# hpcaitech/Open-Sora

Hardware: NVIDIA H100
Metric: denoise-steps/sec STDiT3-XL/2 64x32x32 bf16 (higher is better)
Workload: dtype bf16

## Files before the change

### open-sora_b200/csrc/gemm_sm90.cu

```cuda
#include <stdlib.h>

#include <type_traits>

#include "common.cuh"
#include "tiles.cuh"
#include "wgmma.cuh"

namespace osb {

constexpr int kBlockM = 128;
constexpr int kBlockK = 64;
constexpr int kNumThreads = 384;
constexpr int kStageBudget = 200 * 1024;
constexpr int kSmemLimit = 227 * 1024;

enum { kPlain = 0, kConv = 1, kHeadTiles = 2, kLora = 3, kText = 4, kFp8 = 5, kFp8Blk = 6 };

struct Fp8BlockParams {
  int64_t a_ld, a_kstride;
  uint8_t* d8;
  float* d_scale;
  int64_t ldd8, ld_dscale;
};

// ... 31 lines not shown
  int32_t kw_n, kh_n;
  int32_t cin_chunks;
};

__host__ __device__ constexpr bool staged_epilogue(int mode) { return mode == kPlain || mode == kConv || mode == kLora || mode == kFp8 || mode == kFp8Blk; }

template <int BLOCK_N, bool kStaged = false>
struct GemmCfg {
  static constexpr int A_BYTES = kBlockM * kBlockK * 2;
  static constexpr int B_BYTES = BLOCK_N * kBlockK * 2;
  static constexpr int STAGE_BYTES = A_BYTES + B_BYTES;
  static constexpr int EPI_BYTES = kStaged ? kBlockM * BLOCK_N * 2 : 0;
  static constexpr int RING_BUDGET = kStaged ? kSmemLimit - 1024 - 256 - EPI_BYTES : kStageBudget;
  static constexpr int STAGES_RAW = RING_BUDGET / STAGE_BYTES;
  static constexpr int STAGES = STAGES_RAW > 6 ? 6 : STAGES_RAW;
  static constexpr int NUM_BARS = 2 * STAGES + (kStaged ? 1 : 0);
  static constexpr int SMEM_BYTES = STAGES * STAGE_BYTES + EPI_BYTES + 1024 + 8 * NUM_BARS;
  static_assert(STAGES >= 2, "pipeline needs at least two stages");
  static_assert(SMEM_BYTES <= kSmemLimit, "shared memory");
  static_assert(B_BYTES % 1024 == 0, "W tile must keep 1024-byte swizzle-atom alignment");
  static_assert(BLOCK_N % 16 == 0 && BLOCK_N <= 256, "wgmma N");
  static_assert(!kStaged || BLOCK_N % 64 == 0, "the staged epilogue moves 64-column boxes");
};

template <int BLOCK_N, int kMode>
__global__ void __launch_bounds__(kNumThreads, 1)
gemm_bf16_kernel(const __grid_constant__ CUtensorMap tmap_a, const __grid_constant__ CUtensorMap tmap_w,
                 const GemmEpilogueParams p, const ConvGeom cg, const HeadTileParams ht,
                 const __grid_constant__ CUtensorMap tmap_u, const __grid_constant__ CUtensorMap tmap_lb,
                 const int32_t lora_k_blocks,
                 const float* a_scale, const float* w_scale,
                 const Fp8BlockParams fb,
                 const __grid_constant__ CUtensorMap tmap_r,
                 const __grid_constant__ CUtensorMap tmap_d) {
  constexpr bool kStaged = staged_epilogue(kMode);
  using Cfg = GemmCfg<BLOCK_N, kStaged>;
  constexpr int kStages = Cfg::STAGES;
  constexpr int kBK = (kMode == kFp8 || kMode == kFp8Blk) ? 2 * kBlockK : kBlockK;
  constexpr uint32_t kEpiBoxBytes = kBlockM * 128;

  extern __shared__ uint8_t smem_raw[];
  const uint32_t smem_base = (smem_u32(smem_raw) + 1023u) & ~1023u;
  const uint32_t epi_base = smem_base + kStages * Cfg::STAGE_BYTES;
  const uint32_t bar_base = epi_base + Cfg::EPI_BYTES;
  auto full_bar = [&](int s) { return bar_base + 8u * s; };
  auto empty_bar = [&](int s) { return bar_base + 8u * (kStages + s); };
  const uint32_t res_bar = bar_base + 8u * (2 * kStages);
  auto smem_a = [&](int s) { return smem_base + s * Cfg::STAGE_BYTES; };
  auto smem_b = [&](int s) { return smem_base + s * Cfg::STAGE_BYTES + Cfg::A_BYTES; };

  const int wg = threadIdx.x >> 7;
  const int tid_wg = threadIdx.x & 127;
  const int64_t num_n_blocks = (p.N + BLOCK_N - 1) / BLOCK_N;
  const int64_t m_blk = blockIdx.x / num_n_blocks, n_blk = blockIdx.x % num_n_blocks;
  const int64_t num_k_blocks = (p.K + kBK - 1) / kBK;
  const int64_t total_k_blocks = kMode == kLora ? num_k_blocks + lora_k_blocks : num_k_blocks;
  int n_i = 0, t0 = 0, h0 = 0, w0 = 0;
  if constexpr (kMode == kConv) {
    const int tw = (int)(m_blk % cg.tiles_w);
    const int th = (int)((m_blk / cg.tiles_w) % cg.tiles_h);
    const int tt = (int)((m_blk / ((int64_t)cg.tiles_w * cg.tiles_h)) % cg.tiles_t);
    n_i = (int)(m_blk / ((int64_t)cg.tiles_w * cg.tiles_h * cg.tiles_t));
    w0 = tw << cg.wt_log2;
    h0 = th << cg.ht_log2;
    t0 = tt * (128 >> (cg.wt_log2 + cg.ht_log2));
  }

  if (threadIdx.x == 0) {
    tma_prefetch_desc(&tmap_a);
    tma_prefetch_desc(&tmap_w);
    if constexpr (kMode == kLora) {
      tma_prefetch_desc(&tmap_u);
      tma_prefetch_desc(&tmap_lb);
    }
    if constexpr (kStaged) {
      if (p.R != nullptr) tma_prefetch_desc(&tmap_r);
      tma_prefetch_desc(&tmap_d);
      mbar_init(res_bar, 1);
    }
    for (int s = 0; s < kStages; ++s) {
      mbar_init(full_bar(s), 1);
      mbar_init(empty_bar(s), 2);
    }
    fence_barrier_init();
  }
  __syncthreads();
  pdl_wait();

  if (wg == 0) {
    if (tid_wg == 0) {
      const int32_t a_row = (int32_t)(m_blk * kBlockM);
      const int32_t w_row = (int32_t)(n_blk * BLOCK_N);
      if constexpr (kStaged) {
        if (p.R != nullptr) {
          const int live = (int)min((int64_t)(BLOCK_N / 64), (p.N - w_row + 63) / 64);
          mbar_expect_tx(res_bar, (uint32_t)live * kEpiBoxBytes);
          for (int c = 0; c < live; ++c) {
            if constexpr (kMode == kConv)
              tma_load_5d(&tmap_r, res_bar, epi_base + c * kEpiBoxBytes, w_row + 64 * c, w0, h0, t0, n_i);
            else
              tma_load_2d(&tmap_r, res_bar, epi_base + c * kEpiBoxBytes, w_row + 64 * c, a_row);
          }
        }
      }
      int stage = 0;
      uint32_t phase = 0;
      for (int64_t kb = 0; kb < num_k_blocks; ++kb) {
        mbar_wait_notrace(empty_bar(stage), phase ^ 1);
        const int32_t k0 = (int32_t)(kb * kBK);
        mbar_expect_tx(full_bar(stage), Cfg::STAGE_BYTES);
        if constexpr (kMode == kConv) {
          const int tap = (int)(kb / cg.cin_chunks);
          const int32_t ac = (int32_t)(kb - (int64_t)tap * cg.cin_chunks) * kBlockK;
          const int32_t aw = w0 * cg.sw + tap % cg.kw_n;
          const int32_t ah = h0 * cg.sh + (tap / cg.kw_n) % cg.kh_n;
          const int32_t at = t0 * cg.st + tap / (cg.kw_n * cg.kh_n);
          tma_load_5d(&tmap_a, full_bar(stage), smem_a(stage), ac, aw, ah, at, n_i);
        } else {
          tma_load_2d(&tmap_a, full_bar(stage), smem_a(stage), k0, a_row);
        }
        tma_load_2d(&tmap_w, full_bar(stage), smem_b(stage), k0, w_row);
        if (++stage == kStages) { stage = 0; phase ^= 1; }
      }
      if constexpr (kMode == kLora) {
        for (int32_t lk = 0; lk < lora_k_blocks; ++lk) {
          mbar_wait_notrace(empty_bar(stage), phase ^ 1);
          mbar_expect_tx(full_bar(stage), Cfg::STAGE_BYTES);
          tma_load_2d(&tmap_u, full_bar(stage), smem_a(stage), lk * kBlockK, a_row);
          tma_load_2d(&tmap_lb, full_bar(stage), smem_b(stage), lk * kBlockK, w_row);
          if (++stage == kStages) { stage = 0; phase ^= 1; }
        }
      }
      pdl_launch_dependents();
    }
    return;
  }

  const int cw = wg - 1;
  float acc[BLOCK_N / 2];
#pragma unroll
  for (int i = 0; i < BLOCK_N / 2; ++i) acc[i] = 0.f;
  if constexpr (kMode == kFp8 || kMode == kFp8Blk) {
    float part[BLOCK_N / 2];
#pragma unroll
    for (int i = 0; i < BLOCK_N / 2; ++i) part[i] = 0.f;
    const float* sa_row0 = a_scale;
    const float* sa_row1 = a_scale;
    if constexpr (kMode == kFp8Blk) {
      const int64_t r0 = m_blk * kBlockM + cw * 64 + (tid_wg >> 5) * 16 + ((tid_wg & 31) >> 2);
      sa_row0 = a_scale + min(r0, p.M - 1) * fb.a_ld;
      sa_row1 = a_scale + min(r0 + 8, p.M - 1) * fb.a_ld;
    }
    int stage = 0;
    uint32_t phase = 0;
    for (int64_t kb = 0; kb < total_k_blocks; ++kb) {
      float s0 = 1.f, s1 = 1.f;
      if constexpr (kMode == kFp8Blk) {
        s0 = __ldg(sa_row0 + kb * fb.a_kstride);
        s1 = __ldg(sa_row1 + kb * fb.a_kstride);
      }
      mbar_wait_notrace(full_bar(stage), phase);
      const uint64_t da = make_sw128_kmajor_desc(smem_a(stage) + (uint32_t)(cw * 64 * 128));
      const uint64_t db = make_sw128_kmajor_desc(smem_b(stage));
      wgmma_fence_regs(part);
      wgmma_fence();
#pragma unroll
      for (int k = 0; k < 4; ++k)
        WgmmaFp8<BLOCK_N>::mma(part, da + (uint64_t)(2 * k), db + (uint64_t)(2 * k), k > 0 ? 1u : 0u);
      wgmma_commit();
      wgmma_wait<0>();
      wgmma_fence_regs(part);
      if (tid_wg == 0) mbar_arrive(empty_bar(stage));
      if constexpr (kMode == kFp8Blk) {
#pragma unroll
        for (int j = 0; j < BLOCK_N / 8; ++j) {
          acc[4 * j] = fmaf(part[4 * j], s0, acc[4 * j]);
          acc[4 * j + 1] = fmaf(part[4 * j + 1], s0, acc[4 * j + 1]);
          acc[4 * j + 2] = fmaf(part[4 * j + 2], s1, acc[4 * j + 2]);
          acc[4 * j + 3] = fmaf(part[4 * j + 3], s1, acc[4 * j + 3]);
        }
      } else {
#pragma unroll
        for (int i = 0; i < BLOCK_N / 2; ++i) acc[i] += part[i];
      }
      if (++stage == kStages) { stage = 0; phase ^= 1; }
    }
  } else {
    int stage = 0, prev = 0;
    uint32_t phase = 0;
    for (int64_t kb = 0; kb < total_k_blocks; ++kb) {
      mbar_wait_notrace(full_bar(stage), phase);
      const uint64_t da = make_sw128_kmajor_desc(smem_a(stage) + (uint32_t)(cw * 64 * 128));
      const uint64_t db = make_sw128_kmajor_desc(smem_b(stage));
      wgmma_fence_regs(acc);
      wgmma_fence();
#pragma unroll
      for (int k = 0; k < kBlockK / 16; ++k)
        Wgmma<BLOCK_N>::mma(acc, da + (uint64_t)(2 * k), db + (uint64_t)(2 * k), (kb > 0 || k > 0) ? 1u : 0u);
      wgmma_commit();
      wgmma_wait<1>();
      wgmma_fence_regs(acc);
      if (kb > 0 && tid_wg == 0) mbar_arrive(empty_bar(prev));
      prev = stage;
      if (++stage == kStages) { stage = 0; phase ^= 1; }
    }
    wgmma_wait<0>();
    wgmma_fence_regs(acc);
  }

  const int warp_in = tid_wg >> 5, lane = tid_wg & 31;
  const int r_frag = cw * 64 + warp_in * 16 + (lane >> 2);
  const int c_frag = 2 * (lane & 3);

  if constexpr (kMode == kLora) {
    if (w_scale != nullptr) {
#pragma unroll
      for (int j = 0; j < BLOCK_N / 8; ++j) {
        const int64_t n = min(n_blk * BLOCK_N + 8 * j + c_frag, p.N - 2);
        const float2 cs = __ldg(reinterpret_cast<const float2*>(w_scale + n));
        acc[4 * j] *= cs.x;
        acc[4 * j + 1] *= cs.y;
        acc[4 * j + 2] *= cs.x;
        acc[4 * j + 3] *= cs.y;
      }
    }
  }

  if constexpr (kMode == kFp8Blk && BLOCK_N == 128) {
    if (p.epilogue == OSB_EPI_BIAS_GELU_TANH_FP8) {
      const int64_t n0 = n_blk * BLOCK_N + c_frag;
#pragma unroll
      for (int h = 0; h < 2; ++h) {
        const int64_t row = m_blk * kBlockM + r_frag + 8 * h;
        float amax = 0.f;
#pragma unroll
        for (int j = 0; j < BLOCK_N / 8; ++j) {
          const int64_t n = n0 + 8 * j;
          const float2 sw = __ldg(reinterpret_cast<const float2*>(w_scale + n));
          float v0 = acc[4 * j + 2 * h] * sw.x, v1 = acc[4 * j + 2 * h + 1] * sw.y;
          if (p.bias) {
            const float2 b = unpack_bf16x2(__ldg(reinterpret_cast<const uint32_t*>(p.bias + n)));
            v0 += b.x;
            v1 += b.y;
          }
          v0 = gelu_tanh(v0);
          v1 = gelu_tanh(v1);
          acc[4 * j + 2 * h] = v0;
          acc[4 * j + 2 * h + 1] = v1;
          amax = fmaxf(amax, fmaxf(fabsf(v0), fabsf(v1)));
        }
        amax = fmaxf(amax, __shfl_xor_sync(0xffffffffu, amax, 1));
        amax = fmaxf(amax, __shfl_xor_sync(0xffffffffu, amax, 2));
        const float s = amax > 0.f ? amax / 448.0f : 1.0f;
        if (row < p.M) {
          uint8_t* drow = fb.d8 + row * fb.ldd8;
#pragma unroll
          for (int j = 0; j < BLOCK_N / 8; ++j)
            *reinterpret_cast<uint16_t*>(drow + n0 + 8 * j) =
                (uint16_t)e4m3x2(acc[4 * j + 2 * h] / s, acc[4 * j + 2 * h + 1] / s);
          if (c_frag == 0) fb.d_scale[row * fb.ld_dscale + n_blk] = s;
        }
      }
      return;
    }
  }

  if constexpr (kMode == kHeadTiles) {
    constexpr int D = BLOCK_N / 2;
    using HT = HeadTileCfg<D>;
    constexpr int JH = D / 8;
    const int C = ht.heads * D;
    const uint32_t chunk_bytes = (uint32_t)ht.map.TR * 128u;
#pragma unroll
    for (int h = 0; h < 2; ++h) {
      const int64_t row = m_blk * kBlockM + r_frag + 8 * h;
      const bool row_ok = row < p.M;
      uint32_t pos = 0, tile_i = 0, seq;
      int r = 0;
      if (row_ok) {
        const uint32_t row32 = (uint32_t)row;
        if (ht.map.mode == 0) {
          seq = row32 / (uint32_t)ht.map.L;
          pos = row32 - seq * (uint32_t)ht.map.L;
        } else {
          const uint32_t ts = (uint32_t)ht.map.T * (uint32_t)ht.map.S;
          const uint32_t b = row32 / ts;
          const uint32_t rem = row32 - b * ts;
          pos = rem / (uint32_t)ht.map.S;
          seq = b * (uint32_t)ht.map.S + (rem - pos * (uint32_t)ht.map.S);
        }
        if (ht.map.G > 1) {
          tile_i = seq / (uint32_t)ht.map.G;
          r = (int)((seq - tile_i * (uint32_t)ht.map.G) * (uint32_t)ht.map.L + pos);
        } else {
          const uint32_t jt = pos / (uint32_t)ht.map.TR;
          tile_i = seq * (uint32_t)ht.map.tps + jt;
          r = (int)(pos - jt * (uint32_t)ht.map.TR);
        }
      }
#pragma unroll
      for (int hh = 0; hh < 2; ++hh) {
        const int64_t col0 = n_blk * BLOCK_N + hh * D;
        if (col0 >= p.N) continue;
        const int kidx = (int)((uint32_t)col0 / (uint32_t)C);
        const int head = (int)((uint32_t)col0 - (uint32_t)kidx * (uint32_t)C) / D;
        const int kind = kidx % ht.nkinds;
        float x[JH][2];
#pragma unroll
        for (int j = 0; j < JH; ++j) {
          x[j][0] = acc[4 * (hh * JH + j) + 2 * h];
          x[j][1] = acc[4 * (hh * JH + j) + 2 * h + 1];
          if (p.bias) {
            const float2 b = unpack_bf16x2(__ldg(reinterpret_cast<const uint32_t*>(p.bias + col0 + 8 * j + c_frag)));
            x[j][0] += b.x;
            x[j][1] += b.y;
          }
        }
        if ((ht.norm_mask >> kind) & 1u) {
          float ss = 0.f;
#pragma unroll
          for (int j = 0; j < JH; ++j) ss += x[j][0] * x[j][0] + x[j][1] * x[j][1];
          ss += __shfl_xor_sync(0xffffffffu, ss, 1);
          ss += __shfl_xor_sync(0xffffffffu, ss, 2);
          const float rs = rsqrtf(ss * (1.0f / D) + ht.eps);
          const __nv_bfloat16* w = kind == 0 ? ht.norm_w[0] : (kind == 1 ? ht.norm_w[1] : (kind == 2 ? ht.norm_w[2] : ht.norm_w[3]));
#pragma unroll
          for (int j = 0; j < JH; ++j) {
            const float2 f = unpack_bf16x2(__ldg(reinterpret_cast<const uint32_t*>(w + 8 * j + c_frag)));
            x[j][0] *= rs * f.x;
            x[j][1] *= rs * f.y;
          }
        }
        if (!row_ok) continue;
        if ((ht.rope_mask >> kind) & 1u) {
#pragma unroll
          for (int j = 0; j < JH; ++j) {
            const int64_t i = (int64_t)pos * (D / 2) + (8 * j + c_frag) / 2;
            const float cc = __ldg(ht.cos + i), sn = __ldg(ht.sin + i);
            const float a = x[j][0], b = x[j][1];
            x[j][0] = a * cc - b * sn;
            x[j][1] = b * cc + a * sn;
          }
        }
        uint8_t* dst = ht.base + (int64_t)kidx * ht.kind_stride + (int64_t)head * ht.head_stride + (int64_t)tile_i * ht.tile_bytes;
#pragma unroll
        for (int j = 0; j < JH; ++j)
          *reinterpret_cast<uint32_t*>(dst + tile_unit_off<HT::MAIN>(r, j, chunk_bytes) + c_frag * 2) = pack_bf16x2(x[j][0], x[j][1]);
        if constexpr (HT::UP > HT::U)
          *reinterpret_cast<uint32_t*>(dst + tile_unit_off<HT::MAIN>(r, HT::U, chunk_bytes) + c_frag * 2) = 0u;
      }
    }
  } else if constexpr (kMode == kText) {
#pragma unroll
    for (int h = 0; h < 2; ++h) {
      const int64_t row = m_blk * kBlockM + r_frag + 8 * h;
      if (row >= p.M) continue;
      __nv_bfloat16* drow = p.D + row * p.ldd;
#pragma unroll
      for (int j = 0; j < BLOCK_N / 8; ++j) {
        const int64_t n = n_blk * BLOCK_N + 8 * j + c_frag;
        if (n >= p.N) continue;
        float v0 = acc[4 * j + 2 * h], v1 = acc[4 * j + 2 * h + 1];
        if (p.bias) {
          const float2 b = unpack_bf16x2(__ldg(reinterpret_cast<const uint32_t*>(p.bias + n)));
          v0 += b.x;
          v1 += b.y;
        }
        if (p.epilogue == OSB_EPI_GATED_GELU) {
          drow[n >> 1] = __float2bfloat16_rn(gelu_tanh(v0) * v1);
        } else {
          v0 = v0 / (1.0f + __expf(-1.702f * v0));
          v1 = v1 / (1.0f + __expf(-1.702f * v1));
          *reinterpret_cast<uint32_t*>(drow + n) = pack_bf16x2(v0, v1);
        }
      }
    }
  } else {
    static_assert(kStaged, "every other mode has its own epilogue");
    const float* gate_row[2] = {nullptr, nullptr};
    float sa[2] = {0.f, 0.f};
    if constexpr (kMode != kConv) {
      const uint32_t group_rows32 = (uint32_t)(p.group_rows > 0xffffffffll ? 0xffffffffu : p.group_rows);
#pragma unroll
      for (int h = 0; h < 2; ++h) {
        const int64_t row = min(m_blk * kBlockM + r_frag + 8 * h, p.M - 1);
        if (p.epilogue == OSB_EPI_BIAS_GATE_RES && p.gate != nullptr) {
          int64_t gi = (uint32_t)row / group_rows32;
          if (p.mod_index) gi = p.mod_index[gi];
          gate_row[h] = p.gate + gi * p.gate_stride;
        }
        if constexpr (kMode == kFp8) sa[h] = __ldg(a_scale + row);
      }
    }
    uint8_t* const epi = smem_raw + (epi_base - smem_u32(smem_raw));
    const bool gate_res = p.epilogue == OSB_EPI_BIAS_GATE_RES;
    if (!gate_res) gate_row[0] = gate_row[1] = nullptr;
    const bool has_res = gate_res && p.R != nullptr;
    if (p.R != nullptr) mbar_wait_notrace(res_bar, 0);
    auto body = [&](auto gelu) {
#pragma unroll
      for (int j = 0; j < BLOCK_N / 8; ++j) {
        const int64_t n = min(n_blk * BLOCK_N + 8 * j + c_frag, p.N - 2);
        float2 sw = make_float2(1.f, 1.f), b = make_float2(-0.f, -0.f);
        if constexpr (kMode == kFp8 || kMode == kFp8Blk) sw = __ldg(reinterpret_cast<const float2*>(w_scale + n));
        if (p.bias) b = unpack_bf16x2(__ldg(reinterpret_cast<const uint32_t*>(p.bias + n)));
#pragma unroll
        for (int h = 0; h < 2; ++h) {
          const int li = r_frag + 8 * h;
          uint32_t* const cell = reinterpret_cast<uint32_t*>(epi + (j >> 3) * kEpiBoxBytes + li * 128 +
                                                             (((j & 7) ^ (li & 7)) << 4) + c_frag * 2);
          float v0 = acc[4 * j + 2 * h], v1 = acc[4 * j + 2 * h + 1];
          if constexpr (kMode == kFp8) {
            v0 = __fmul_rn(v0, __fmul_rn(sa[h], sw.x));
            v1 = __fmul_rn(v1, __fmul_rn(sa[h], sw.y));
          } else if constexpr (kMode == kFp8Blk) {
            v0 = __fmul_rn(v0, sw.x);
            v1 = __fmul_rn(v1, sw.y);
          }
          v0 = __fadd_rn(v0, b.x);
          v1 = __fadd_rn(v1, b.y);
          if constexpr (decltype(gelu)::value) {
            v0 = gelu_tanh(v0);
            v1 = gelu_tanh(v1);
          } else {
            const float2 g = gate_row[h] ? __ldg(reinterpret_cast<const float2*>(gate_row[h] + n)) : make_float2(1.f, 1.f);
            const float2 rv = has_res ? unpack_bf16x2(*cell) : make_float2(-0.f, -0.f);
            v0 = __fadd_rn(__fmul_rn(v0, g.x), rv.x);
            v1 = __fadd_rn(__fmul_rn(v1, g.y), rv.y);
          }
          *cell = pack_bf16x2(v0, v1);
        }
      }
    };
    if (p.epilogue == OSB_EPI_BIAS_GELU_TANH)
      body(std::true_type{});
    else
      body(std::false_type{});
    fence_proxy_async_smem();
    named_barrier_sync(1, 256);
    if (threadIdx.x == 128) {
      const int32_t n0 = (int32_t)(n_blk * BLOCK_N);
      const int live = (int)min((int64_t)(BLOCK_N / 64), (p.N - n0 + 63) / 64);
      for (int c = 0; c < live; ++c) {
        if constexpr (kMode == kConv)
          tma_store_5d(&tmap_d, epi_base + c * kEpiBoxBytes, n0 + 64 * c, w0, h0, t0, n_i);
        else
          tma_store_2d(&tmap_d, epi_base + c * kEpiBoxBytes, n0 + 64 * c, (int32_t)(m_blk * kBlockM));
      }
      bulk_commit_group();
      bulk_wait_group_read_all();
    }
  }
}

template <int BLOCK_N, int kMode>
static int launch_kernel(const CUtensorMap& ta, const CUtensorMap& tw, const GemmEpilogueParams& p, const ConvGeom& cg,
                         const HeadTileParams& ht, int64_t tiles, cudaStream_t stream, const CUtensorMap* tu = nullptr,
                         const CUtensorMap* tlb = nullptr, int32_t lora_k_blocks = 0, const float* a_scale = nullptr,
                         const float* w_scale = nullptr, const Fp8BlockParams& fb = Fp8BlockParams{},
                         const CUtensorMap* tr = nullptr, const CUtensorMap* td = nullptr) {
  if (tiles >= (1ll << 31)) { set_error("osb gemm: too many output tiles (%lld)", (long long)tiles); return OSB_ERR_UNSUPPORTED; }
  cudaLaunchAttribute attr[2];
  cudaLaunchConfig_t cfg = launch_config(dim3((unsigned)tiles), dim3(kNumThreads),
                                         GemmCfg<BLOCK_N, staged_epilogue(kMode)>::SMEM_BYTES, stream, attr);
  OSB_CHECK_CUDA(cudaLaunchKernelEx(&cfg, gemm_bf16_kernel<BLOCK_N, kMode>, ta, tw, p, cg, ht, tu ? *tu : ta,
                                    tlb ? *tlb : tw, lora_k_blocks, a_scale, w_scale, fb, tr ? *tr : ta, td ? *td : ta));
  count_launch();
  return OSB_OK;
}

static int make_epilogue_maps(const GemmEpilogueParams& p, CUtensorMap* tr, CUtensorMap* td) {
  if (int rc = make_tmap_2d_bf16(td, p.D, p.M, p.N, p.ldd, kBlockM, 64)) return rc;
  if (p.R != nullptr) return make_tmap_2d_bf16(tr, p.R, p.M, p.N, p.ldr, kBlockM, 64);
  *tr = *td;
  return OSB_OK;
}

template <int D>
static int launch_gemm_ht(const osb_gemm_args& a, const HeadTileParams& ht, cudaStream_t stream) {
  constexpr int BLOCK_N = 2 * D;
  CUtensorMap ta, tw;
  int rc = make_tmap_2d_bf16(&ta, a.A, a.M, a.K, a.lda, kBlockM, kBlockK);
  if (rc) return rc;
  rc = make_tmap_2d_bf16(&tw, a.W, a.N, a.K, a.ldw, BLOCK_N, kBlockK);
  if (rc) return rc;
  GemmEpilogueParams p = {};
  p.bias = static_cast<const __nv_bfloat16*>(a.bias);
  p.M = a.M; p.N = a.N; p.K = a.K;
  p.group_rows = a.M;
  p.epilogue = OSB_EPI_BIAS;
  const int64_t tiles = ((a.M + kBlockM - 1) / kBlockM) * ((a.N + BLOCK_N - 1) / BLOCK_N);
  ConvGeom cg = {};
  return launch_kernel<BLOCK_N, kHeadTiles>(ta, tw, p, cg, ht, tiles, stream);
}

template <int BLOCK_N>
static int launch_gemm(const osb_gemm_args& a, bool has_res, cudaStream_t stream, const osb_lora_args* lora = nullptr) {
  CUtensorMap ta, tw;
  int rc = make_tmap_2d_bf16(&ta, a.A, a.M, a.K, a.lda, kBlockM, kBlockK);
// ... 405 lines not shown
```

Before: 11.21.

## Make SM90 GEMM persistent with a tile loop and register reallocation

Converts the warp-specialized GEMM into a persistent kernel. The grid is capped at the SM count, and each CTA loops over output tiles while the producer keeps the TMA stage ring running across tile boundaries. The residual prefetch moves to a consumer thread and is issued after the first wgmma of each tile, once prior epilogue stores have drained. setmaxnreg shifts registers from the producer warpgroup to the consumers. This removes per-tile launch and prologue cost and lets the next tile's loads overlap the current epilogue, at the cost of more complex barrier and phase handling and possible tail imbalance.

```diff
diff --git a/open-sora_b200/csrc/gemm_sm90.cu b/open-sora_b200/csrc/gemm_sm90.cu
--- a/open-sora_b200/csrc/gemm_sm90.cu
+++ b/open-sora_b200/csrc/gemm_sm90.cu
@@ -87,7 +87,8 @@
                  const float* a_scale, const float* w_scale,
                  const Fp8BlockParams fb,
                  const __grid_constant__ CUtensorMap tmap_r,
-                 const __grid_constant__ CUtensorMap tmap_d) {
+                 const __grid_constant__ CUtensorMap tmap_d,
+                 const int32_t num_tiles) {
   constexpr bool kStaged = staged_epilogue(kMode);
   using Cfg = GemmCfg<BLOCK_N, kStaged>;
   constexpr int kStages = Cfg::STAGES;
@@ -107,19 +108,28 @@
   const int wg = threadIdx.x >> 7;
   const int tid_wg = threadIdx.x & 127;
   const int64_t num_n_blocks = (p.N + BLOCK_N - 1) / BLOCK_N;
-  const int64_t m_blk = blockIdx.x / num_n_blocks, n_blk = blockIdx.x % num_n_blocks;
   const int64_t num_k_blocks = (p.K + kBK - 1) / kBK;
   const int64_t total_k_blocks = kMode == kLora ? num_k_blocks + lora_k_blocks : num_k_blocks;
-  int n_i = 0, t0 = 0, h0 = 0, w0 = 0;
-  if constexpr (kMode == kConv) {
-    const int tw = (int)(m_blk % cg.tiles_w);
-    const int th = (int)((m_blk / cg.tiles_w) % cg.tiles_h);
-    const int tt = (int)((m_blk / ((int64_t)cg.tiles_w * cg.tiles_h)) % cg.tiles_t);
-    n_i = (int)(m_blk / ((int64_t)cg.tiles_w * cg.tiles_h * cg.tiles_t));
-    w0 = tw << cg.wt_log2;
-    h0 = th << cg.ht_log2;
-    t0 = tt * (128 >> (cg.wt_log2 + cg.ht_log2));
-  }
+  struct Tile {
+    int32_t m_blk, n_blk;
+    int n_i, t0, h0, w0;
+  };
+  auto tile_at = [&](uint32_t t) {
+    Tile c;
+    c.m_blk = (int32_t)(t / (uint32_t)num_n_blocks);
+    c.n_blk = (int32_t)(t % (uint32_t)num_n_blocks);
+    c.n_i = c.t0 = c.h0 = c.w0 = 0;
+    if constexpr (kMode == kConv) {
+      const int tw = (int)(c.m_blk % cg.tiles_w);
+      const int th = (int)((c.m_blk / cg.tiles_w) % cg.tiles_h);
+      const int tt = (int)((c.m_blk / ((int64_t)cg.tiles_w * cg.tiles_h)) % cg.tiles_t);
+      c.n_i = (int)(c.m_blk / ((int64_t)cg.tiles_w * cg.tiles_h * cg.tiles_t));
+      c.w0 = tw << cg.wt_log2;
+      c.h0 = th << cg.ht_log2;
+      c.t0 = tt * (128 >> (cg.wt_log2 + cg.ht_log2));
+    }
+    return c;
+  };
 
   if (threadIdx.x == 0) {
     tma_prefetch_desc(&tmap_a);
@@ -143,369 +153,386 @@
   pdl_wait();
 
   if (wg == 0) {
+    asm volatile("setmaxnreg.dec.sync.aligned.u32 40;\n" ::: "memory");
     if (tid_wg == 0) {
-      const int32_t a_row = (int32_t)(m_blk * kBlockM);
-      const int32_t w_row = (int32_t)(n_blk * BLOCK_N);
+      int stage = 0;
+      uint32_t phase = 0;
+      for (uint32_t tile = blockIdx.x; tile < (uint32_t)num_tiles; tile += gridDim.x) {
+        const Tile c = tile_at(tile);
+        const int32_t a_row = (int32_t)(c.m_blk * kBlockM);
+        const int32_t w_row = (int32_t)(c.n_blk * BLOCK_N);
+        for (int64_t kb = 0; kb < num_k_blocks; ++kb) {
+          mbar_wait_notrace(empty_bar(stage), phase ^ 1);
+          const int32_t k0 = (int32_t)(kb * kBK);
+          mbar_expect_tx(full_bar(stage), Cfg::STAGE_BYTES);
+          if constexpr (kMode == kConv) {
+            const int tap = (int)(kb / cg.cin_chunks);
+            const int32_t ac = (int32_t)(kb - (int64_t)tap * cg.cin_chunks) * kBlockK;
+            const int32_t aw = c.w0 * cg.sw + tap % cg.kw_n;
+            const int32_t ah = c.h0 * cg.sh + (tap / cg.kw_n) % cg.kh_n;
+            const int32_t at = c.t0 * cg.st + tap / (cg.kw_n * cg.kh_n);
+            tma_load_5d(&tmap_a, full_bar(stage), smem_a(stage), ac, aw, ah, at, c.n_i);
+          } else {
+            tma_load_2d(&tmap_a, full_bar(stage), smem_a(stage), k0, a_row);
+          }
+          tma_load_2d(&tmap_w, full_bar(stage), smem_b(stage), k0, w_row);
+          if (++stage == kStages) { stage = 0; phase ^= 1; }
+        }
+        if constexpr (kMode == kLora) {
+          for (int32_t lk = 0; lk < lora_k_blocks; ++lk) {
+            mbar_wait_notrace(empty_bar(stage), phase ^ 1);
+            mbar_expect_tx(full_bar(stage), Cfg::STAGE_BYTES);
+            tma_load_2d(&tmap_u, full_bar(stage), smem_a(stage), lk * kBlockK, a_row);
+            tma_load_2d(&tmap_lb, full_bar(stage), smem_b(stage), lk * kBlockK, w_row);
+            if (++stage == kStages) { stage = 0; phase ^= 1; }
+          }
+        }
+      }
+      pdl_launch_dependents();
+    }
+    return;
+  }
+
+  asm volatile("setmaxnreg.inc.sync.aligned.u32 232;\n" ::: "memory");
+  const int cw = wg - 1;
+  const int warp_in = tid_wg >> 5, lane = tid_wg & 31;
+  const int r_frag = cw * 64 + warp_in * 16 + (lane >> 2);
+  const int c_frag = 2 * (lane & 3);
+  int stage = 0;
+  uint32_t phase = 0;
+  uint32_t it = 0;
+  for (uint32_t tile = blockIdx.x; tile < (uint32_t)num_tiles; tile += gridDim.x, ++it) {
+    const Tile tc = tile_at(tile);
+    const int64_t m_blk = tc.m_blk, n_blk = tc.n_blk;
+    auto refill_epilogue_buffer = [&]() {
       if constexpr (kStaged) {
+        bulk_wait_group_read_all();
         if (p.R != nullptr) {
+          const int32_t w_row = (int32_t)(n_blk * BLOCK_N);
           const int live = (int)min((int64_t)(BLOCK_N / 64), (p.N - w_row + 63) / 64);
           mbar_expect_tx(res_bar, (uint32_t)live * kEpiBoxBytes);
           for (int c = 0; c < live; ++c) {
             if constexpr (kMode == kConv)
-              tma_load_5d(&tmap_r, res_bar, epi_base + c * kEpiBoxBytes, w_row + 64 * c, w0, h0, t0, n_i);
+              tma_load_5d(&tmap_r, res_bar, epi_base + c * kEpiBoxBytes, w_row + 64 * c, tc.w0, tc.h0, tc.t0, tc.n_i);
             else
-              tma_load_2d(&tmap_r, res_bar, epi_base + c * kEpiBoxBytes, w_row + 64 * c, a_row);
-          }
-        }
-      }
-      int stage = 0;
-      uint32_t phase = 0;
-      for (int64_t kb = 0; kb < num_k_blocks; ++kb) {
-        mbar_wait_notrace(empty_bar(stage), phase ^ 1);
-        const int32_t k0 = (int32_t)(kb * kBK);
-        mbar_expect_tx(full_bar(stage), Cfg::STAGE_BYTES);
-        if constexpr (kMode == kConv) {
-          const int tap = (int)(kb / cg.cin_chunks);
-          const int32_t ac = (int32_t)(kb - (int64_t)tap * cg.cin_chunks) * kBlockK;
-          const int32_t aw = w0 * cg.sw + tap % cg.kw_n;
-          const int32_t ah = h0 * cg.sh + (tap / cg.kw_n) % cg.kh_n;
-          const int32_t at = t0 * cg.st + tap / (cg.kw_n * cg.kh_n);
-          tma_load_5d(&tmap_a, full_bar(stage), smem_a(stage), ac, aw, ah, at, n_i);
+              tma_load_2d(&tmap_r, res_bar, epi_base + c * kEpiBoxBytes, w_row + 64 * c, (int32_t)(m_blk * kBlockM));
+          }
+        }
+      }
+    };
+    float acc[BLOCK_N / 2];
+#pragma unroll
+    for (int i = 0; i < BLOCK_N / 2; ++i) acc[i] = 0.f;
+    if constexpr (kMode == kFp8 || kMode == kFp8Blk) {
+      float part[BLOCK_N / 2];
+#pragma unroll
+      for (int i = 0; i < BLOCK_N / 2; ++i) part[i] = 0.f;
+      const float* sa_row0 = a_scale;
+      const float* sa_row1 = a_scale;
+      if constexpr (kMode == kFp8Blk) {
+        const int64_t r0 = m_blk * kBlockM + cw * 64 + (tid_wg >> 5) * 16 + ((tid_wg & 31) >> 2);
+        sa_row0 = a_scale + min(r0, p.M - 1) * fb.a_ld;
+        sa_row1 = a_scale + min(r0 + 8, p.M - 1) * fb.a_ld;
+      }
+      for (int64_t kb = 0; kb < total_k_blocks; ++kb) {
+        float s0 = 1.f, s1 = 1.f;
+        if constexpr (kMode == kFp8Blk) {
+          s0 = __ldg(sa_row0 + kb * fb.a_kstride);
+          s1 = __ldg(sa_row1 + kb * fb.a_kstride);
+        }
+        mbar_wait_notrace(full_bar(stage), phase);
+        const uint64_t da = make_sw128_kmajor_desc(smem_a(stage) + (uint32_t)(cw * 64 * 128));
+        const uint64_t db = make_sw128_kmajor_desc(smem_b(stage));
+        wgmma_fence_regs(part);
+        wgmma_fence();
+#pragma unroll
+        for (int k = 0; k < 4; ++k)
+          WgmmaFp8<BLOCK_N>::mma(part, da + (uint64_t)(2 * k), db + (uint64_t)(2 * k), k > 0 ? 1u : 0u);
+        wgmma_commit();
+        if (kb == 0 && threadIdx.x == 128) refill_epilogue_buffer();
+        wgmma_wait<0>();
+        wgmma_fence_regs(part);
+        if (tid_wg == 0) mbar_arrive(empty_bar(stage));
+        if constexpr (kMode == kFp8Blk) {
+#pragma unroll
+          for (int j = 0; j < BLOCK_N / 8; ++j) {
+            acc[4 * j] = fmaf(part[4 * j], s0, acc[4 * j]);
+            acc[4 * j + 1] = fmaf(part[4 * j + 1], s0, acc[4 * j + 1]);
+            acc[4 * j + 2] = fmaf(part[4 * j + 2], s1, acc[4 * j + 2]);
+            acc[4 * j + 3] = fmaf(part[4 * j + 3], s1, acc[4 * j + 3]);
+          }
         } else {
-          tma_load_2d(&tmap_a, full_bar(stage), smem_a(stage), k0, a_row);
-        }
-        tma_load_2d(&tmap_w, full_bar(stage), smem_b(stage), k0, w_row);
+#pragma unroll
+          for (int i = 0; i < BLOCK_N / 2; ++i) acc[i] += part[i];
+        }
         if (++stage == kStages) { stage = 0; phase ^= 1; }
       }
-      if constexpr (kMode == kLora) {
-        for (int32_t lk = 0; lk < lora_k_blocks; ++lk) {
-          mbar_wait_notrace(empty_bar(stage), phase ^ 1);
-          mbar_expect_tx(full_bar(stage), Cfg::STAGE_BYTES);
-          tma_load_2d(&tmap_u, full_bar(stage), smem_a(stage), lk * kBlockK, a_row);
-          tma_load_2d(&tmap_lb, full_bar(stage), smem_b(stage), lk * kBlockK, w_row);
-          if (++stage == kStages) { stage = 0; phase ^= 1; }
-        }
-      }
-      pdl_launch_dependents();
+    } else {
+      int prev = 0;
+      for (int64_t kb = 0; kb < total_k_blocks; ++kb) {
+        mbar_wait_notrace(full_bar(stage), phase);
+        const uint64_t da = make_sw128_kmajor_desc(smem_a(stage) + (uint32_t)(cw * 64 * 128));
+        const uint64_t db = make_sw128_kmajor_desc(smem_b(stage));
+        wgmma_fence_regs(acc);
+        wgmma_fence();
+#pragma unroll
+        for (int k = 0; k < kBlockK / 16; ++k)
+          Wgmma<BLOCK_N>::mma(acc, da + (uint64_t)(2 * k), db + (uint64_t)(2 * k), (kb > 0 || k > 0) ? 1u : 0u);
+        wgmma_commit();
+        if (kb == 0 && threadIdx.x == 128) refill_epilogue_buffer();
+        wgmma_wait<1>();
+        wgmma_fence_regs(acc);
+        if (kb > 0 && tid_wg == 0) mbar_arrive(empty_bar(prev));
+        prev = stage;
+        if (++stage == kStages) { stage = 0; phase ^= 1; }
+      }
+      wgmma_wait<0>();
+      wgmma_fence_regs(acc);
+      if (tid_wg == 0) mbar_arrive(empty_bar(prev));
     }
-    return;
-  }
-
-  const int cw = wg - 1;
-  float acc[BLOCK_N / 2];
-#pragma unroll
-  for (int i = 0; i < BLOCK_N / 2; ++i) acc[i] = 0.f;
-  if constexpr (kMode == kFp8 || kMode == kFp8Blk) {
-    float part[BLOCK_N / 2];
-#pragma unroll
-    for (int i = 0; i < BLOCK_N / 2; ++i) part[i] = 0.f;
-    const float* sa_row0 = a_scale;
-    const float* sa_row1 = a_scale;
-    if constexpr (kMode == kFp8Blk) {
-      const int64_t r0 = m_blk * kBlockM + cw * 64 + (tid_wg >> 5) * 16 + ((tid_wg & 31) >> 2);
-      sa_row0 = a_scale + min(r0, p.M - 1) * fb.a_ld;
-      sa_row1 = a_scale + min(r0 + 8, p.M - 1) * fb.a_ld;
+
+    if constexpr (kMode == kLora) {
+      if (w_scale != nullptr) {
+#pragma unroll
+        for (int j = 0; j < BLOCK_N / 8; ++j) {
+          const int64_t n = min(n_blk * BLOCK_N + 8 * j + c_frag, p.N - 2);
+          const float2 cs = __ldg(reinterpret_cast<const float2*>(w_scale + n));
+          acc[4 * j] *= cs.x;
+          acc[4 * j + 1] *= cs.y;
+          acc[4 * j + 2] *= cs.x;
+          acc[4 * j + 3] *= cs.y;
+        }
+      }
     }
-    int stage = 0;
-    uint32_t phase = 0;
-    for (int64_t kb = 0; kb < total_k_blocks; ++kb) {
-      float s0 = 1.f, s1 = 1.f;
-      if constexpr (kMode == kFp8Blk) {
-        s0 = __ldg(sa_row0 + kb * fb.a_kstride);
-        s1 = __ldg(sa_row1 + kb * fb.a_kstride);
-      }
-      mbar_wait_notrace(full_bar(stage), phase);
-      const uint64_t da = make_sw128_kmajor_desc(smem_a(stage) + (uint32_t)(cw * 64 * 128));
-      const uint64_t db = make_sw128_kmajor_desc(smem_b(stage));
-      wgmma_fence_regs(part);
-      wgmma_fence();
-#pragma unroll
-      for (int k = 0; k < 4; ++k)
-        WgmmaFp8<BLOCK_N>::mma(part, da + (uint64_t)(2 * k), db + (uint64_t)(2 * k), k > 0 ? 1u : 0u);
-      wgmma_commit();
-      wgmma_wait<0>();
-      wgmma_fence_regs(part);
-      if (tid_wg == 0) mbar_arrive(empty_bar(stage));
-      if constexpr (kMode == kFp8Blk) {
-#pragma unroll
-        for (int j = 0; j < BLOCK_N / 8; ++j) {
-          acc[4 * j] = fmaf(part[4 * j], s0, acc[4 * j]);
-          acc[4 * j + 1] = fmaf(part[4 * j + 1], s0, acc[4 * j + 1]);
-          acc[4 * j + 2] = fmaf(part[4 * j + 2], s1, acc[4 * j + 2]);
-          acc[4 * j + 3] = fmaf(part[4 * j + 3], s1, acc[4 * j + 3]);
-        }
-      } else {
-#pragma unroll
-        for (int i = 0; i < BLOCK_N / 2; ++i) acc[i] += part[i];
-      }
-      if (++stage == kStages) { stage = 0; phase ^= 1; }
+
+    if constexpr (kMode == kFp8Blk && BLOCK_N == 128) {
+      if (p.epilogue == OSB_EPI_BIAS_GELU_TANH_FP8) {
+        const int64_t n0 = n_blk * BLOCK_N + c_frag;
+#pragma unroll
+        for (int h = 0; h < 2; ++h) {
+          const int64_t row = m_blk * kBlockM + r_frag + 8 * h;
+          float amax = 0.f;
+#pragma unroll
+          for (int j = 0; j < BLOCK_N / 8; ++j) {
+            const int64_t n = n0 + 8 * j;
+            const float2 sw = __ldg(reinterpret_cast<const float2*>(w_scale + n));
+            float v0 = acc[4 * j + 2 * h] * sw.x, v1 = acc[4 * j + 2 * h + 1] * sw.y;
+            if (p.bias) {
+              const float2 b = unpack_bf16x2(__ldg(reinterpret_cast<const uint32_t*>(p.bias + n)));
+              v0 += b.x;
+              v1 += b.y;
+            }
+            v0 = gelu_tanh(v0);
+            v1 = gelu_tanh(v1);
+            acc[4 * j + 2 * h] = v0;
+            acc[4 * j + 2 * h + 1] = v1;
+            amax = fmaxf(amax, fmaxf(fabsf(v0), fabsf(v1)));
+          }
+          amax = fmaxf(amax, __shfl_xor_sync(0xffffffffu, amax, 1));
+          amax = fmaxf(amax, __shfl_xor_sync(0xffffffffu, amax, 2));
+          const float s = amax > 0.f ? amax / 448.0f : 1.0f;
+          if (row < p.M) {
+            uint8_t* drow = fb.d8 + row * fb.ldd8;
+#pragma unroll
+            for (int j = 0; j < BLOCK_N / 8; ++j)
+              *reinterpret_cast<uint16_t*>(drow + n0 + 8 * j) =
+                  (uint16_t)e4m3x2(acc[4 * j + 2 * h] / s, acc[4 * j + 2 * h + 1] / s);
+            if (c_frag == 0) fb.d_scale[row * fb.ld_dscale + n_blk] = s;
+          }
+        }
+        continue;
+      }
     }
-  } else {
-    int stage = 0, prev = 0;
-    uint32_t phase = 0;
-    for (int64_t kb = 0; kb < total_k_blocks; ++kb) {
-      mbar_wait_notrace(full_bar(stage), phase);
-      const uint64_t da = make_sw128_kmajor_desc(smem_a(stage) + (uint32_t)(cw * 64 * 128));
-      const uint64_t db = make_sw128_kmajor_desc(smem_b(stage));
-      wgmma_fence_regs(acc);
-      wgmma_fence();
-#pragma unroll
-      for (int k = 0; k < kBlockK / 16; ++k)
-        Wgmma<BLOCK_N>::mma(acc, da + (uint64_t)(2 * k), db + (uint64_t)(2 * k), (kb > 0 || k > 0) ? 1u : 0u);
-      wgmma_commit();
-      wgmma_wait<1>();
-      wgmma_fence_regs(acc);
-      if (kb > 0 && tid_wg == 0) mbar_arrive(empty_bar(prev));
-      prev = stage;
-      if (++stage == kStages) { stage = 0; phase ^= 1; }
-    }
-    wgmma_wait<0>();
-    wgmma_fence_regs(acc);
-  }
-
-  const int warp_in = tid_wg >> 5, lane = tid_wg & 31;
-  const int r_frag = cw * 64 + warp_in * 16 + (lane >> 2);
-  const int c_frag = 2 * (lane & 3);
-
-  if constexpr (kMode == kLora) {
-    if (w_scale != nullptr) {
-#pragma unroll
-      for (int j = 0; j < BLOCK_N / 8; ++j) {
-        const int64_t n = min(n_blk * BLOCK_N + 8 * j + c_frag, p.N - 2);
-        const float2 cs = __ldg(reinterpret_cast<const float2*>(w_scale + n));
-        acc[4 * j] *= cs.x;
-        acc[4 * j + 1] *= cs.y;
-        acc[4 * j + 2] *= cs.x;
-        acc[4 * j + 3] *= cs.y;
-      }
-    }
-  }
-
-  if constexpr (kMode == kFp8Blk && BLOCK_N == 128) {
-    if (p.epilogue == OSB_EPI_BIAS_GELU_TANH_FP8) {
-      const int64_t n0 = n_blk * BLOCK_N + c_frag;
+
+    if constexpr (kMode == kHeadTiles) {
+      constexpr int D = BLOCK_N / 2;
+      using HT = HeadTileCfg<D>;
+      constexpr int JH = D / 8;
+      const int C = ht.heads * D;
+      const uint32_t chunk_bytes = (uint32_t)ht.map.TR * 128u;
 #pragma unroll
       for (int h = 0; h < 2; ++h) {
         const int64_t row = m_blk * kBlockM + r_frag + 8 * h;
-        float amax = 0.f;
+        const bool row_ok = row < p.M;
+        uint32_t pos = 0, tile_i = 0, seq;
+        int r = 0;
+        if (row_ok) {
+          const uint32_t row32 = (uint32_t)row;
+          if (ht.map.mode == 0) {
+            seq = row32 / (uint32_t)ht.map.L;
+            pos = row32 - seq * (uint32_t)ht.map.L;
+          } else {
+            const uint32_t ts = (uint32_t)ht.map.T * (uint32_t)ht.map.S;
+            const uint32_t b = row32 / ts;
+            const uint32_t rem = row32 - b * ts;
+            pos = rem / (uint32_t)ht.map.S;
+            seq = b * (uint32_t)ht.map.S + (rem - pos * (uint32_t)ht.map.S);
+          }
+          if (ht.map.G > 1) {
+            tile_i = seq / (uint32_t)ht.map.G;
+            r = (int)((seq - tile_i * (uint32_t)ht.map.G) * (uint32_t)ht.map.L + pos);
+          } else {
+            const uint32_t jt = pos / (uint32_t)ht.map.TR;
+            tile_i = seq * (uint32_t)ht.map.tps + jt;
+            r = (int)(pos - jt * (uint32_t)ht.map.TR);
+          }
+        }
+#pragma unroll
+        for (int hh = 0; hh < 2; ++hh) {
+          const int64_t col0 = n_blk * BLOCK_N + hh * D;
+          if (col0 >= p.N) continue;
+          const int kidx = (int)((uint32_t)col0 / (uint32_t)C);
+          const int head = (int)((uint32_t)col0 - (uint32_t)kidx * (uint32_t)C) / D;
+          const int kind = kidx % ht.nkinds;
+          float x[JH][2];
+#pragma unroll
+          for (int j = 0; j < JH; ++j) {
+            x[j][0] = acc[4 * (hh * JH + j) + 2 * h];
+            x[j][1] = acc[4 * (hh * JH + j) + 2 * h + 1];
+            if (p.bias) {
+              const float2 b = unpack_bf16x2(__ldg(reinterpret_cast<const uint32_t*>(p.bias + col0 + 8 * j + c_frag)));
+              x[j][0] += b.x;
+              x[j][1] += b.y;
+            }
+          }
+          if ((ht.norm_mask >> kind) & 1u) {
+            float ss = 0.f;
+#pragma unroll
+            for (int j = 0; j < JH; ++j) ss += x[j][0] * x[j][0] + x[j][1] * x[j][1];
+            ss += __shfl_xor_sync(0xffffffffu, ss, 1);
+            ss += __shfl_xor_sync(0xffffffffu, ss, 2);
+            const float rs = rsqrtf(ss * (1.0f / D) + ht.eps);
+            const __nv_bfloat16* w = kind == 0 ? ht.norm_w[0] : (kind == 1 ? ht.norm_w[1] : (kind == 2 ? ht.norm_w[2] : ht.norm_w[3]));
+#pragma unroll
+            for (int j = 0; j < JH; ++j) {
+              const float2 f = unpack_bf16x2(__ldg(reinterpret_cast<const uint32_t*>(w + 8 * j + c_frag)));
+              x[j][0] *= rs * f.x;
+              x[j][1] *= rs * f.y;
+            }
+          }
+          if (!row_ok) continue;
+          if ((ht.rope_mask >> kind) & 1u) {
+#pragma unroll
+            for (int j = 0; j < JH; ++j) {
+              const int64_t i = (int64_t)pos * (D / 2) + (8 * j + c_frag) / 2;
+              const float cc = __ldg(ht.cos + i), sn = __ldg(ht.sin + i);
+              const float a = x[j][0], b = x[j][1];
+              x[j][0] = a * cc - b * sn;
+              x[j][1] = b * cc + a * sn;
+            }
+          }
+          uint8_t* dst = ht.base + (int64_t)kidx * ht.kind_stride + (int64_t)head * ht.head_stride + (int64_t)tile_i * ht.tile_bytes;
+#pragma unroll
+          for (int j = 0; j < JH; ++j)
+            *reinterpret_cast<uint32_t*>(dst + tile_unit_off<HT::MAIN>(r, j, chunk_bytes) + c_frag * 2) = pack_bf16x2(x[j][0], x[j][1]);
+          if constexpr (HT::UP > HT::U)
+            *reinterpret_cast<uint32_t*>(dst + tile_unit_off<HT::MAIN>(r, HT::U, chunk_bytes) + c_frag * 2) = 0u;
+        }
+      }
+    } else if constexpr (kMode == kText) {
+#pragma unroll
+      for (int h = 0; h < 2; ++h) {
+        const int64_t row = m_blk * kBlockM + r_frag + 8 * h;
+        if (row >= p.M) continue;
+        __nv_bfloat16* drow = p.D + row * p.ldd;
 #pragma unroll
         for (int j = 0; j < BLOCK_N / 8; ++j) {
-          const int64_t n = n0 + 8 * j;
-          const float2 sw = __ldg(reinterpret_cast<const float2*>(w_scale + n));
-          float v0 = acc[4 * j + 2 * h] * sw.x, v1 = acc[4 * j + 2 * h + 1] * sw.y;
+          const int64_t n = n_blk * BLOCK_N + 8 * j + c_frag;
+          if (n >= p.N) continue;
+          float v0 = acc[4 * j + 2 * h], v1 = acc[4 * j + 2 * h + 1];
           if (p.bias) {
             const float2 b = unpack_bf16x2(__ldg(reinterpret_cast<const uint32_t*>(p.bias + n)));
             v0 += b.x;
             v1 += b.y;
           }
-          v0 = gelu_tanh(v0);
-          v1 = gelu_tanh(v1);
-          acc[4 * j + 2 * h] = v0;
-          acc[4 * j + 2 * h + 1] = v1;
-          amax = fmaxf(amax, fmaxf(fabsf(v0), fabsf(v1)));
-        }
-        amax = fmaxf(amax, __shfl_xor_sync(0xffffffffu, amax, 1));
-        amax = fmaxf(amax, __shfl_xor_sync(0xffffffffu, amax, 2));
-        const float s = amax > 0.f ? amax / 448.0f : 1.0f;
-        if (row < p.M) {
-          uint8_t* drow = fb.d8 + row * fb.ldd8;
-#pragma unroll
-          for (int j = 0; j < BLOCK_N / 8; ++j)
-            *reinterpret_cast<uint16_t*>(drow + n0 + 8 * j) =
-                (uint16_t)e4m3x2(acc[4 * j + 2 * h] / s, acc[4 * j + 2 * h + 1] / s);
-          if (c_frag == 0) fb.d_scale[row * fb.ld_dscale + n_blk] = s;
-        }
-      }
-      return;
+          if (p.epilogue == OSB_EPI_GATED_GELU) {
+            drow[n >> 1] = __float2bfloat16_rn(gelu_tanh(v0) * v1);
+          } else {
+            v0 = v0 / (1.0f + __expf(-1.702f * v0));
+            v1 = v1 / (1.0f + __expf(-1.702f * v1));
+            *reinterpret_cast<uint32_t*>(drow + n) = pack_bf16x2(v0, v1);
+          }
+        }
+      }
+    } else {
+      static_assert(kStaged, "every other mode has its own epilogue");
+      const float* gate_row[2] = {nullptr, nullptr};
+      float sa[2] = {0.f, 0.f};
+      if constexpr (kMode != kConv) {
+        const uint32_t group_rows32 = (uint32_t)(p.group_rows > 0xffffffffll ? 0xffffffffu : p.group_rows);
+#pragma unroll
+        for (int h = 0; h < 2; ++h) {
+          const int64_t row = min(m_blk * kBlockM + r_frag + 8 * h, p.M - 1);
+          if (p.epilogue == OSB_EPI_BIAS_GATE_RES && p.gate != nullptr) {
+            int64_t gi = (uint32_t)row / group_rows32;
+            if (p.mod_index) gi = p.mod_index[gi];
+            gate_row[h] = p.gate + gi * p.gate_stride;
+          }
+          if constexpr (kMode == kFp8) sa[h] = __ldg(a_scale + row);
+        }
+      }
+      uint8_t* const epi = smem_raw + (epi_base - smem_u32(smem_raw));
+      const bool gate_res = p.epilogue == OSB_EPI_BIAS_GATE_RES;
+      if (!gate_res) gate_row[0] = gate_row[1] = nullptr;
+      const bool has_res = gate_res && p.R != nullptr;
+      named_barrier_sync(1, 256);
+      if (p.R != nullptr) mbar_wait_notrace(res_bar, it & 1u);
+      auto body = [&](auto gelu) {
+#pragma unroll
+        for (int j = 0; j < BLOCK_N / 8; ++j) {
+          const int64_t n = min(n_blk * BLOCK_N + 8 * j + c_frag, p.N - 2);
+          float2 sw = make_float2(1.f, 1.f), b = make_float2(-0.f, -0.f);
+          if constexpr (kMode == kFp8 || kMode == kFp8Blk) sw = __ldg(reinterpret_cast<const float2*>(w_scale + n));
+          if (p.bias) b = unpack_bf16x2(__ldg(reinterpret_cast<const uint32_t*>(p.bias + n)));
+#pragma unroll
+          for (int h = 0; h < 2; ++h) {
+            const int li = r_frag + 8 * h;
+            uint32_t* const cell = reinterpret_cast<uint32_t*>(epi + (j >> 3) * kEpiBoxBytes + li * 128 +
+                                                               (((j & 7) ^ (li & 7)) << 4) + c_frag * 2);
+            float v0 = acc[4 * j + 2 * h], v1 = acc[4 * j + 2 * h + 1];
+            if constexpr (kMode == kFp8) {
+              v0 = __fmul_rn(v0, __fmul_rn(sa[h], sw.x));
+              v1 = __fmul_rn(v1, __fmul_rn(sa[h], sw.y));
+            } else if constexpr (kMode == kFp8Blk) {
+              v0 = __fmul_rn(v0, sw.x);
+              v1 = __fmul_rn(v1, sw.y);
+            }
+            v0 = __fadd_rn(v0, b.x);
+            v1 = __fadd_rn(v1, b.y);
+            if constexpr (decltype(gelu)::value) {
+              v0 = gelu_tanh(v0);
+              v1 = gelu_tanh(v1);
+            } else {
+              const float2 g = gate_row[h] ? __ldg(reinterpret_cast<const float2*>(gate_row[h] + n)) : make_float2(1.f, 1.f);
+              const float2 rv = has_res ? unpack_bf16x2(*cell) : make_float2(-0.f, -0.f);
+              v0 = __fadd_rn(__fmul_rn(v0, g.x), rv.x);
+              v1 = __fadd_rn(__fmul_rn(v1, g.y), rv.y);
+            }
+            *cell = pack_bf16x2(v0, v1);
+          }
+        }
+      };
+      if (p.epilogue == OSB_EPI_BIAS_GELU_TANH)
+        body(std::true_type{});
+      else
+        body(std::false_type{});
+      fence_proxy_async_smem();
+      named_barrier_sync(1, 256);
+      if (threadIdx.x == 128) {
+        const int32_t n0 = (int32_t)(n_blk * BLOCK_N);
+        const int live = (int)min((int64_t)(BLOCK_N / 64), (p.N - n0 + 63) / 64);
+        for (int c = 0; c < live; ++c) {
+          if constexpr (kMode == kConv)
+            tma_store_5d(&tmap_d, epi_base + c * kEpiBoxBytes, n0 + 64 * c, tc.w0, tc.h0, tc.t0, tc.n_i);
+          else
+            tma_store_2d(&tmap_d, epi_base + c * kEpiBoxBytes, n0 + 64 * c, (int32_t)(m_blk * kBlockM));
+        }
+        bulk_commit_group();
+      }
     }
   }
-
-  if constexpr (kMode == kHeadTiles) {
-    constexpr int D = BLOCK_N / 2;
-    using HT = HeadTileCfg<D>;
-    constexpr int JH = D / 8;
-    const int C = ht.heads * D;
-    const uint32_t chunk_bytes = (uint32_t)ht.map.TR * 128u;
-#pragma unroll
-    for (int h = 0; h < 2; ++h) {
-      const int64_t row = m_blk * kBlockM + r_frag + 8 * h;
-      const bool row_ok = row < p.M;
-      uint32_t pos = 0, tile_i = 0, seq;
-      int r = 0;
-      if (row_ok) {
-        const uint32_t row32 = (uint32_t)row;
-        if (ht.map.mode == 0) {
-          seq = row32 / (uint32_t)ht.map.L;
-          pos = row32 - seq * (uint32_t)ht.map.L;
-        } else {
-          const uint32_t ts = (uint32_t)ht.map.T * (uint32_t)ht.map.S;
-          const uint32_t b = row32 / ts;
-          const uint32_t rem = row32 - b * ts;
-          pos = rem / (uint32_t)ht.map.S;
-          seq = b * (uint32_t)ht.map.S + (rem - pos * (uint32_t)ht.map.S);
-        }
-        if (ht.map.G > 1) {
-          tile_i = seq / (uint32_t)ht.map.G;
-          r = (int)((seq - tile_i * (uint32_t)ht.map.G) * (uint32_t)ht.map.L + pos);
-        } else {
-          const uint32_t jt = pos / (uint32_t)ht.map.TR;
-          tile_i = seq * (uint32_t)ht.map.tps + jt;
-          r = (int)(pos - jt * (uint32_t)ht.map.TR);
-        }
-      }
-#pragma unroll
-      for (int hh = 0; hh < 2; ++hh) {
-        const int64_t col0 = n_blk * BLOCK_N + hh * D;
-        if (col0 >= p.N) continue;
-        const int kidx = (int)((uint32_t)col0 / (uint32_t)C);
-        const int head = (int)((uint32_t)col0 - (uint32_t)kidx * (uint32_t)C) / D;
-        const int kind = kidx % ht.nkinds;
-        float x[JH][2];
-#pragma unroll
-        for (int j = 0; j < JH; ++j) {
-          x[j][0] = acc[4 * (hh * JH + j) + 2 * h];
-          x[j][1] = acc[4 * (hh * JH + j) + 2 * h + 1];
-          if (p.bias) {
-            const float2 b = unpack_bf16x2(__ldg(reinterpret_cast<const uint32_t*>(p.bias + col0 + 8 * j + c_frag)));
-            x[j][0] += b.x;
-            x[j][1] += b.y;
-          }
-        }
-        if ((ht.norm_mask >> kind) & 1u) {
-          float ss = 0.f;
-#pragma unroll
-          for (int j = 0; j < JH; ++j) ss += x[j][0] * x[j][0] + x[j][1] * x[j][1];
-          ss += __shfl_xor_sync(0xffffffffu, ss, 1);
-          ss += __shfl_xor_sync(0xffffffffu, ss, 2);
-          const float rs = rsqrtf(ss * (1.0f / D) + ht.eps);
-          const __nv_bfloat16* w = kind == 0 ? ht.norm_w[0] : (kind == 1 ? ht.norm_w[1] : (kind == 2 ? ht.norm_w[2] : ht.norm_w[3]));
-#pragma unroll
-          for (int j = 0; j < JH; ++j) {
-            const float2 f = unpack_bf16x2(__ldg(reinterpret_cast<const uint32_t*>(w + 8 * j + c_frag)));
-            x[j][0] *= rs * f.x;
-            x[j][1] *= rs * f.y;
-          }
-        }
-        if (!row_ok) continue;
-        if ((ht.rope_mask >> kind) & 1u) {
-#pragma unroll
-          for (int j = 0; j < JH; ++j) {
-            const int64_t i = (int64_t)pos * (D / 2) + (8 * j + c_frag) / 2;
-            const float cc = __ldg(ht.cos + i), sn = __ldg(ht.sin + i);
-            const float a = x[j][0], b = x[j][1];
-            x[j][0] = a * cc - b * sn;
-            x[j][1] = b * cc + a * sn;
-          }
-        }
-        uint8_t* dst = ht.base + (int64_t)kidx * ht.kind_stride + (int64_t)head * ht.head_stride + (int64_t)tile_i * ht.tile_bytes;
-#pragma unroll
-        for (int j = 0; j < JH; ++j)
-          *reinterpret_cast<uint32_t*>(dst + tile_unit_off<HT::MAIN>(r, j, chunk_bytes) + c_frag * 2) = pack_bf16x2(x[j][0], x[j][1]);
-        if constexpr (HT::UP > HT::U)
-          *reinterpret_cast<uint32_t*>(dst + tile_unit_off<HT::MAIN>(r, HT::U, chunk_bytes) + c_frag * 2) = 0u;
-      }
-    }
-  } else if constexpr (kMode == kText) {
-#pragma unroll
-    for (int h = 0; h < 2; ++h) {
-      const int64_t row = m_blk * kBlockM + r_frag + 8 * h;
-      if (row >= p.M) continue;
-      __nv_bfloat16* drow = p.D + row * p.ldd;
-#pragma unroll
-      for (int j = 0; j < BLOCK_N / 8; ++j) {
-        const int64_t n = n_blk * BLOCK_N + 8 * j + c_frag;
-        if (n >= p.N) continue;
-        float v0 = acc[4 * j + 2 * h], v1 = acc[4 * j + 2 * h + 1];
-        if (p.bias) {
-          const float2 b = unpack_bf16x2(__ldg(reinterpret_cast<const uint32_t*>(p.bias + n)));
-          v0 += b.x;
-          v1 += b.y;
-        }
-        if (p.epilogue == OSB_EPI_GATED_GELU) {
-          drow[n >> 1] = __float2bfloat16_rn(gelu_tanh(v0) * v1);
-        } else {
-          v0 = v0 / (1.0f + __expf(-1.702f * v0));
-          v1 = v1 / (1.0f + __expf(-1.702f * v1));
-          *reinterpret_cast<uint32_t*>(drow + n) = pack_bf16x2(v0, v1);
-        }
-      }
-    }
-  } else {
-    static_assert(kStaged, "every other mode has its own epilogue");
-    const float* gate_row[2] = {nullptr, nullptr};
-    float sa[2] = {0.f, 0.f};
-    if constexpr (kMode != kConv) {
-      const uint32_t group_rows32 = (uint32_t)(p.group_rows > 0xffffffffll ? 0xffffffffu : p.group_rows);
-#pragma unroll
-      for (int h = 0; h < 2; ++h) {
-        const int64_t row = min(m_blk * kBlockM + r_frag + 8 * h, p.M - 1);
-        if (p.epilogue == OSB_EPI_BIAS_GATE_RES && p.gate != nullptr) {
-          int64_t gi = (uint32_t)row / group_rows32;
-          if (p.mod_index) gi = p.mod_index[gi];
-          gate_row[h] = p.gate + gi * p.gate_stride;
-        }
-        if constexpr (kMode == kFp8) sa[h] = __ldg(a_scale + row);
-      }
-    }
-    uint8_t* const epi = smem_raw + (epi_base - smem_u32(smem_raw));
-    const bool gate_res = p.epilogue == OSB_EPI_BIAS_GATE_RES;
-    if (!gate_res) gate_row[0] = gate_row[1] = nullptr;
-    const bool has_res = gate_res && p.R != nullptr;
-    if (p.R != nullptr) mbar_wait_notrace(res_bar, 0);
-    auto body = [&](auto gelu) {
-#pragma unroll
-      for (int j = 0; j < BLOCK_N / 8; ++j) {
-        const int64_t n = min(n_blk * BLOCK_N + 8 * j + c_frag, p.N - 2);
-        float2 sw = make_float2(1.f, 1.f), b = make_float2(-0.f, -0.f);
-        if constexpr (kMode == kFp8 || kMode == kFp8Blk) sw = __ldg(reinterpret_cast<const float2*>(w_scale + n));
-        if (p.bias) b = unpack_bf16x2(__ldg(reinterpret_cast<const uint32_t*>(p.bias + n)));
-#pragma unroll
-        for (int h = 0; h < 2; ++h) {
-          const int li = r_frag + 8 * h;
-          uint32_t* const cell = reinterpret_cast<uint32_t*>(epi + (j >> 3) * kEpiBoxBytes + li * 128 +
-                                                             (((j & 7) ^ (li & 7)) << 4) + c_frag * 2);
-          float v0 = acc[4 * j + 2 * h], v1 = acc[4 * j + 2 * h + 1];
-          if constexpr (kMode == kFp8) {
-            v0 = __fmul_rn(v0, __fmul_rn(sa[h], sw.x));
-            v1 = __fmul_rn(v1, __fmul_rn(sa[h], sw.y));
-          } else if constexpr (kMode == kFp8Blk) {
-            v0 = __fmul_rn(v0, sw.x);
-            v1 = __fmul_rn(v1, sw.y);
-          }
-          v0 = __fadd_rn(v0, b.x);
-          v1 = __fadd_rn(v1, b.y);
-          if constexpr (decltype(gelu)::value) {
-            v0 = gelu_tanh(v0);
-            v1 = gelu_tanh(v1);
-          } else {
-            const float2 g = gate_row[h] ? __ldg(reinterpret_cast<const float2*>(gate_row[h] + n)) : make_float2(1.f, 1.f);
-            const float2 rv = has_res ? unpack_bf16x2(*cell) : make_float2(-0.f, -0.f);
-            v0 = __fadd_rn(__fmul_rn(v0, g.x), rv.x);
-            v1 = __fadd_rn(__fmul_rn(v1, g.y), rv.y);
-          }
-          *cell = pack_bf16x2(v0, v1);
-        }
-      }
-    };
-    if (p.epilogue == OSB_EPI_BIAS_GELU_TANH)
-      body(std::true_type{});
-    else
-      body(std::false_type{});
-    fence_proxy_async_smem();
-    named_barrier_sync(1, 256);
-    if (threadIdx.x == 128) {
-      const int32_t n0 = (int32_t)(n_blk * BLOCK_N);
-      const int live = (int)min((int64_t)(BLOCK_N / 64), (p.N - n0 + 63) / 64);
-      for (int c = 0; c < live; ++c) {
-        if constexpr (kMode == kConv)
-          tma_store_5d(&tmap_d, epi_base + c * kEpiBoxBytes, n0 + 64 * c, w0, h0, t0, n_i);
-        else
-          tma_store_2d(&tmap_d, epi_base + c * kEpiBoxBytes, n0 + 64 * c, (int32_t)(m_blk * kBlockM));
-      }
-      bulk_commit_group();
-      bulk_wait_group_read_all();
-    }
-  }
+  if constexpr (kStaged)
+    if (threadIdx.x == 128) bulk_wait_group_read_all();
 }
 
 template <int BLOCK_N, int kMode>
@@ -516,10 +543,12 @@
                          const CUtensorMap* tr = nullptr, const CUtensorMap* td = nullptr) {
   if (tiles >= (1ll << 31)) { set_error("osb gemm: too many output tiles (%lld)", (long long)tiles); return OSB_ERR_UNSUPPORTED; }
   cudaLaunchAttribute attr[2];
-  cudaLaunchConfig_t cfg = launch_config(dim3((unsigned)tiles), dim3(kNumThreads),
+  const int64_t grid = tiles < sm_count() ? tiles : sm_count();
+  cudaLaunchConfig_t cfg = launch_config(dim3((unsigned)grid), dim3(kNumThreads),
                                          GemmCfg<BLOCK_N, staged_epilogue(kMode)>::SMEM_BYTES, stream, attr);
   OSB_CHECK_CUDA(cudaLaunchKernelEx(&cfg, gemm_bf16_kernel<BLOCK_N, kMode>, ta, tw, p, cg, ht, tu ? *tu : ta,
-                                    tlb ? *tlb : tw, lora_k_blocks, a_scale, w_scale, fb, tr ? *tr : ta, td ? *td : ta));
+                                    tlb ? *tlb : tw, lora_k_blocks, a_scale, w_scale, fb, tr ? *tr : ta, td ? *td : ta,
+                                    (int32_t)tiles));
   count_launch();
   return OSB_OK;
 }
```

Measured after the change: 11.35, median of 6. 1.2% higher.
